# endernewton/tf-faster-rcnn

Hardware: AMD Instinct MI355X
Metric: images/sec (600×1000) ResNet-101 Faster R-CNN at 1/2/4/8 MI355X (higher is better)
Workload: dtype f32 (operands, accumulators, results; GEMMs with Cin, Cout % 128 == 0 form each f32 product from two-piece fp16 operands with an exact power-of-two scale per 128-k block on the fp16 matrix pipe -- 3 MFMAs / product, dropped terms <= 3 * 2^-22, measured error vs float64 below the f32-MFMA kernel's; o

## Files before the change

scratch/wino2_time.py:

```python
import os, sys, statistics
ROOT = os.path.dirname(os.path.dirname(os.path.abspath(__file__)))
sys.path.insert(0, os.path.join(ROOT, "tf-faster-rcnn_amd")); sys.path.insert(0, os.path.join(ROOT, "tf-faster-rcnn_amd", "lib"))
import torch
from frcnn_hip import ops
dev = torch.device("cuda:0")
N, H, W, C = 8, 150, 250, 64
g = torch.Generator(device=dev); g.manual_seed(1)
x = (torch.randn(N, H, W, C, device=dev, generator=g).clamp_(min=0) * torch.exp(torch.rand(N, H, W, 1, device=dev, generator=g) * 4 - 2)).contiguous()
w = (torch.randn(3, 3, C, C, device=dev, generator=g) / 24).cpu().numpy()
u = torch.from_numpy(ops.winograd_filter_transform(w, m=2)).to(dev)
planes = ops.gemm_x3_pack(u)
b = torch.randn(C, device=dev, generator=g)
T = ops.winograd_tiles(N, H, W, 2)
v = torch.empty(16, T, C, device=dev); mm = torch.empty(16, T, C, device=dev)
y0 = torch.empty(N, H, W, C, device=dev); y1 = torch.empty(N, H, W, C, device=dev)
def ev(): return torch.cuda.Event(enable_timing=True)
def timed(fn):
    a, z = ev(), ev(); a.record(); fn(); z.record(); return a, z
R = {"fused": [], "wino_in": [], "gemm_x3": [], "wino_out": []}
for it in range(60):
    e = {}
    e["wino_in"] = timed(lambda: ops.winograd_input_transform(x, v, 2))
    e["gemm_x3"] = timed(lambda: ops.gemm_x3(v, planes, 16, T, C, C, out=mm))
    e["wino_out"] = timed(lambda: ops.winograd_output_transform(mm, b, 1, y0, 2))
    e["fused"] = timed(lambda: ops.winograd2_conv_x3(x, planes, b, 1, y1))
    torch.cuda.synchronize()
    if it >= 10:
        for k, (a, z) in e.items(): R[k].append(a.elapsed_time(z) * 1000.0)
print("bit equal at the bench shape:", torch.equal(y0.view(torch.int32), y1.view(torch.int32)))
for k in ("wino_in", "gemm_x3", "wino_out", "fused"):
    print("%-9s median %7.1f us   min %7.1f us   (n = %d)" % (k, statistics.median(R[k]), min(R[k]), len(R[k])))
print("three launches: median sum %.1f us" % sum(statistics.median(R[k]) for k in ("wino_in", "gemm_x3", "wino_out")))
```

tf-faster-rcnn_amd/csrc/winograd2_fused.hip:

```cpp
#include "common.h"
#include "x3_mma.h"

namespace {

constexpr int W2_RUN = 64, W2_C = 64, W2_NT = 256;
constexpr int W2_V_BYTES = W2_RUN * W2_C * 4;
constexpr int W2_P_BYTES = W2_C * W2_C * 2;
constexpr int W2_U_BYTES = 3 * W2_P_BYTES;
constexpr int W2_LDS = 2 * W2_V_BYTES + 2 * W2_U_BYTES;
constexpr int W2_ITEMS = W2_RUN * (W2_C / 4) / W2_NT;
constexpr unsigned W2_OOB = 0x80000000u;

__device__ __forceinline__ int w2_first(int p) { return p == 0 ? 0 : (p == 2 ? 2 : 1); }
__device__ __forceinline__ int w2_second(int p) { return p == 0 ? 2 : (p == 1 ? 2 : (p == 2 ? 1 : 3)); }

__device__ __forceinline__ float4 w2_pm(const float4 a, const float4 b, bool sub) {
  const float4 c = sub ? make_float4(-b.x, -b.y, -b.z, -b.w) : b;
  return make_float4(a.x + c.x, a.y + c.y, a.z + c.z, a.w + c.w);
}

struct Wino2Params {
  const float* x; const unsigned short* up; const float* bias; float* y;
  int N, H, W, TH, TW, T, act;
};

__global__ __launch_bounds__(W2_NT) void k_wino2_conv_x3(const Wino2Params p) {
  extern __shared__ __attribute__((aligned(16))) char smem[];
  const int tid = threadIdx.x, lane = tid & 63;
  const int wave = __builtin_amdgcn_readfirstlane(tid >> 6);
  const int run0 = blockIdx.x * W2_RUN;
  const int H = p.H, W = p.W;

  const int c4 = tid & 15;
  int off0[W2_ITEMS];
  unsigned ok[W2_ITEMS];
#pragma unroll
  for (int r = 0; r < W2_ITEMS; ++r) {
    const int t = run0 + (tid >> 4) + 16 * r, tc = min(t, p.T - 1);
    const int tx = tc % p.TW, ty = (tc / p.TW) % p.TH, img = tc / (p.TW * p.TH);
    const int ih0 = 2 * ty - 1, iw0 = 2 * tx - 1;
    unsigned m = 0;
#pragma unroll
    for (int i = 0; i < 4; ++i) {
      m |= ((unsigned)(ih0 + i) < (unsigned)H ? 1u : 0u) << i;
      m |= ((unsigned)(iw0 + i) < (unsigned)W ? 1u : 0u) << (4 + i);
    }
    ok[r] = t < p.T ? m : 0u;
    off0[r] = (((img * H + ih0) * W + iw0) * W2_C + c4 * 4) * 4;
  }
  const auto xr = __builtin_amdgcn_make_buffer_rsrc((void*)p.x, 0, p.N * H * W * W2_C * 4, 0x00020000);
  auto tap = [&](int r, int i, int j) {
    const bool in = ((ok[r] >> i) & (ok[r] >> (4 + j)) & 1u) != 0;
    const unsigned o = in ? (unsigned)(off0[r] + (i * W + j) * (W2_C * 4)) : W2_OOB;
    return __builtin_bit_cast(float4, __builtin_amdgcn_raw_buffer_load_b128(xr, (int)o, 0, 0));
  };
  float4 d[W2_ITEMS][4][4];
  auto load_column = [&](int j) {
#pragma unroll
    for (int r = 0; r < W2_ITEMS; ++r)
#pragma unroll
      for (int i = 0; i < 4; ++i) d[r][i][j] = tap(r, i, j);
  };
  load_column(0); load_column(2); load_column(1);
  auto form_v = [&](int xi, int nu, int r, int buf) {
    const int ia = w2_first(xi), ib = w2_second(xi), ja = w2_first(nu), jb = w2_second(nu);
    const bool rsub = xi != 1, csub = nu != 1;
    const float4 ba = w2_pm(d[r][ia][ja], d[r][ib][ja], rsub), bb = w2_pm(d[r][ia][jb], d[r][ib][jb], rsub);
    const int row = (tid >> 4) + 16 * r;
    *(float4*)(smem + buf * W2_V_BYTES + row * (W2_C * 4) + ((c4 ^ (row & 15)) * 16)) = w2_pm(ba, bb, csub);
  };

  const unsigned lds0 = (unsigned)(size_t)(LDS_AS char*)smem;
  int u_lane[2];
#pragma unroll
  for (int t = 0; t < 2; ++t) u_lane[t] = (lane >> 3) * (W2_C * 2) + (((lane & 7) ^ ((4 * t + (lane >> 4)) & 7)) * 16);
  auto load_u = [&](int g, int buf) {
    const char* src = (const char*)p.up + g * W2_U_BYTES + wave * 6 * 1024;
#pragma unroll
    for (int t = 0; t < 6; ++t)
      glds16(src + t * 1024 + u_lane[t & 1], __builtin_amdgcn_readfirstlane(lds0 + 2 * W2_V_BYTES + buf * W2_U_BYTES + (wave * 6 + t) * 1024));
  };

  const int tb = wave >> 1, cb = wave & 1;
  const int frow = lane & 31, khalf = lane >> 5;
  const int a_row = (tb * 32 + frow) * (W2_C * 4), a_sw = frow & 15;
  const int b_row = (cb * 32 + frow) * (W2_C * 2), b_sw = (frow >> 1) & 7;
  f32x16 s0, s1, o[2][2];

  load_u(0, 0);
#pragma unroll
  for (int r = 0; r < W2_ITEMS; ++r) form_v(0, 0, r, 0);
  wait_vmcnt<0>();
  __syncthreads();

#pragma unroll
  for (int nu = 0; nu < 4; ++nu) {
#pragma unroll
    for (int xi = 0; xi < 4; ++xi) {
      const int buf = xi & 1;
      const int nxi = (xi + 1) & 3, nnu = xi == 3 ? nu + 1 : nu;
      const bool more = xi < 3 || nu < 3;
      if (more) load_u(nxi * 4 + nnu, buf ^ 1);
      if (nu == 0 && xi == 3) load_column(3);
      f32x16 acc, acs;
#pragma unroll
      for (int r = 0; r < 16; ++r) { acc[r] = 0.f; acs[r] = 0.f; }
      const char* va = smem + buf * W2_V_BYTES + a_row;
      const char* ub = smem + 2 * W2_V_BYTES + buf * W2_U_BYTES + b_row;
#pragma unroll
      for (int q = 0; q < 4; ++q) {
        bf16x8 ah, am, al;
        const float4 f0 = *(const float4*)(va + (((4 * q + 2 * khalf) ^ a_sw) * 16));
        const float4 f1 = *(const float4*)(va + (((4 * q + 2 * khalf + 1) ^ a_sw) * 16));
        const char* qb = ub + (((2 * q + khalf) ^ b_sw) * 16);
        const bf16x8 bh = __builtin_bit_cast(bf16x8, *(const uint4*)(qb));
        const bf16x8 bm = __builtin_bit_cast(bf16x8, *(const uint4*)(qb + W2_P_BYTES));
        const bf16x8 bl = __builtin_bit_cast(bf16x8, *(const uint4*)(qb + 2 * W2_P_BYTES));
        x3_split8(f0, f1, ah, am, al);
        x3_mma16<6>(ah, am, al, bh, bm, bl, acc, acs);
        if (more) form_v(nxi, nnu, q, buf ^ 1);
      }
      f32x16 m;
#pragma unroll
      for (int r = 0; r < 16; ++r) m[r] = x3_combine_plain(acc[r], acs[r]);
      if (xi == 0) s0 = m;
      if (xi == 1) { s0 = s0 + m; s1 = m; }
      if (xi == 2) { s0 = s0 + m; s1 = s1 - m; }
      if (xi == 3) {
        s1 = s1 - m;
        if (nu == 0) { o[0][0] = s0; o[1][0] = s1; }
        if (nu == 1) { o[0][0] = o[0][0] + s0; o[1][0] = o[1][0] + s1; o[0][1] = s0; o[1][1] = s1; }
        if (nu == 2) { o[0][0] = o[0][0] + s0; o[1][0] = o[1][0] + s1; o[0][1] = o[0][1] - s0; o[1][1] = o[1][1] - s1; }
        if (nu == 3) { o[0][1] = o[0][1] - s0; o[1][1] = o[1][1] - s1; }
      }
      asm volatile("" : "+v"(s0));
      if (xi >= 1) asm volatile("" : "+v"(s1));
      if (xi == 3) {
        if (nu < 3) asm volatile("" : "+v"(o[0][0]), "+v"(o[1][0]));
        if (nu > 0) asm volatile("" : "+v"(o[0][1]), "+v"(o[1][1]));
      }
      wait_vmcnt<0>();
      __syncthreads();
    }
  }

  const int ch = cb * 32 + frow;
  const float bv = p.bias ? p.bias[ch] : 0.f;
  const bool relu = p.act == FRCNN_ACT_RELU;
  int t = run0 + tb * 32 + 4 * khalf;
  int tx = t % p.TW, ty = (t / p.TW) % p.TH, img = t / (p.TW * p.TH);
  auto next_tile = [&]() {
    ++t; ++tx;
    const bool wx = tx == p.TW;
    tx = wx ? 0 : tx; ty += wx ? 1 : 0;
    const bool wy = ty == p.TH;
    ty = wy ? 0 : ty; img += wy ? 1 : 0;
  };
#pragma unroll
  for (int r = 0; r < 16; ++r) {
    if (r) {
#pragma unroll
      for (int k = 0; k < ((r & 3) ? 1 : 5); ++k) next_tile();
    }
    if (t < p.T) {
#pragma unroll
      for (int a = 0; a < 2; ++a)
#pragma unroll
        for (int b = 0; b < 2; ++b) {
          const int oh = 2 * ty + a, ow = 2 * tx + b;
          if (oh >= H || ow >= W) continue;
          float v = o[a][b][r] + bv;
          if (relu) v = act_relu(v);
          p.y[((img * H + oh) * W + ow) * W2_C + ch] = v;
        }
    }
  }
}

}

extern "C" int frcnn_winograd2_conv_x3(const float* x_d, int N, int H, int W, const void* u_planes_d, const float* bias_d, int act,
                                       float* y_d, void* stream) {
  if (!x_d || !u_planes_d || !y_d || N <= 0 || H <= 0 || W <= 0) return FRCNN_E_ARG;
  if (act != FRCNN_ACT_NONE && act != FRCNN_ACT_RELU) return FRCNN_E_UNSUPPORTED;
  if ((long long)N * H * W * W2_C * 4 >= (1ll << 31)) return FRCNN_E_UNSUPPORTED;
  Wino2Params p;
  p.x = x_d; p.up = (const unsigned short*)u_planes_d; p.bias = bias_d; p.y = y_d;
  p.N = N; p.H = H; p.W = W; p.TH = (H + 1) / 2; p.TW = (W + 1) / 2; p.T = N * p.TH * p.TW; p.act = act;
  static KernelOnce once;
  HIP_TRY(kernel_once(once, (const void*)k_wino2_conv_x3, W2_NT, W2_LDS));
  hipLaunchKernelGGL(k_wino2_conv_x3, dim3((unsigned)cdiv(p.T, W2_RUN)), dim3(W2_NT), W2_LDS, (hipStream_t)stream, p);
  LAUNCH_CHECK();
  return FRCNN_OK;
}
```

Before: 563.1.

## Tile fused Winograd F(2,3) conv as 8x8 spatial blocks with LDS halo staging

Each block now owns an 8x8 tile patch of one image rather than a linear run of 64 tiles. It loads the 18x18 input halo once into LDS, split into odd and even column planes, instead of issuing overlapping 4x4 global tap loads per tile. The V operand is split into fp16 hi/mid/lo planes once when written to LDS rather than on every fragment read, and fragments are double-buffered with sched_group_barrier interleaving. Outputs are staged through LDS and written as coalesced float4 rows. This adds LDS pressure and wastes work on edge blocks, and the change also extends the timing script to compare external builds.

```diff
diff --git a/scratch/wino2_time.py b/scratch/wino2_time.py
--- a/scratch/wino2_time.py
+++ b/scratch/wino2_time.py
@@ -1,4 +1,4 @@
-import os, sys, statistics
+import ctypes, os, sys, statistics
 ROOT = os.path.dirname(os.path.dirname(os.path.abspath(__file__)))
 sys.path.insert(0, os.path.join(ROOT, "tf-faster-rcnn_amd")); sys.path.insert(0, os.path.join(ROOT, "tf-faster-rcnn_amd", "lib"))
 import torch
@@ -17,17 +17,29 @@
 def ev(): return torch.cuda.Event(enable_timing=True)
 def timed(fn):
     a, z = ev(), ev(); a.record(); fn(); z.record(); return a, z
-R = {"fused": [], "wino_in": [], "gemm_x3": [], "wino_out": []}
+others = {}
+for path in sys.argv[1:]:
+    L = ctypes.CDLL(os.path.abspath(path)); f = L.frcnn_winograd2_conv_x3; f.restype = ctypes.c_int
+    f.argtypes = [ctypes.c_void_p, ctypes.c_int, ctypes.c_int, ctypes.c_int] + [ctypes.c_void_p] * 2 + [ctypes.c_int] + [ctypes.c_void_p] * 2
+    others["fused@" + os.path.basename(os.path.dirname(os.path.abspath(path)))] = f
+y2 = torch.empty(N, H, W, C, device=dev)
+def other(f):
+    rc = f(x.data_ptr(), N, H, W, planes.data_ptr(), b.data_ptr(), 1, y2.data_ptr(), torch.cuda.current_stream().cuda_stream)
+    assert rc == 0, rc
+R = {k: [] for k in ["fused", "wino_in", "gemm_x3", "wino_out"] + list(others)}
 for it in range(60):
     e = {}
     e["wino_in"] = timed(lambda: ops.winograd_input_transform(x, v, 2))
     e["gemm_x3"] = timed(lambda: ops.gemm_x3(v, planes, 16, T, C, C, out=mm))
     e["wino_out"] = timed(lambda: ops.winograd_output_transform(mm, b, 1, y0, 2))
     e["fused"] = timed(lambda: ops.winograd2_conv_x3(x, planes, b, 1, y1))
+    for k, f in others.items(): e[k] = timed(lambda: other(f))
     torch.cuda.synchronize()
     if it >= 10:
         for k, (a, z) in e.items(): R[k].append(a.elapsed_time(z) * 1000.0)
 print("bit equal at the bench shape:", torch.equal(y0.view(torch.int32), y1.view(torch.int32)))
-for k in ("wino_in", "gemm_x3", "wino_out", "fused"):
+for k, f in others.items():
+    y2.zero_(); other(f); print("%s bit equal to the three launches: %s" % (k, torch.equal(y0.view(torch.int32), y2.view(torch.int32))))
+for k in ["wino_in", "gemm_x3", "wino_out", "fused"] + list(others):
     print("%-9s median %7.1f us   min %7.1f us   (n = %d)" % (k, statistics.median(R[k]), min(R[k]), len(R[k])))
 print("three launches: median sum %.1f us" % sum(statistics.median(R[k]) for k in ("wino_in", "gemm_x3", "wino_out")))
diff --git a/tf-faster-rcnn_amd/csrc/winograd2_fused.hip b/tf-faster-rcnn_amd/csrc/winograd2_fused.hip
--- a/tf-faster-rcnn_amd/csrc/winograd2_fused.hip
+++ b/tf-faster-rcnn_amd/csrc/winograd2_fused.hip
@@ -3,11 +3,17 @@
 
 namespace {
 
-constexpr int W2_RUN = 64, W2_C = 64, W2_NT = 256;
-constexpr int W2_V_BYTES = W2_RUN * W2_C * 4;
+constexpr int W2_BT = 8, W2_RUN = W2_BT * W2_BT, W2_C = 64, W2_NT = 256;
+constexpr int W2_PS = 2 * W2_BT + 2;
 constexpr int W2_P_BYTES = W2_C * W2_C * 2;
-constexpr int W2_U_BYTES = 3 * W2_P_BYTES;
-constexpr int W2_LDS = 2 * W2_V_BYTES + 2 * W2_U_BYTES;
+constexpr int W2_V_BYTES = 3 * W2_P_BYTES, W2_U_BYTES = 3 * W2_P_BYTES;
+constexpr int W2_PLANE = 42 * 1024;
+constexpr int W2_ODD = 0, W2_EVEN = W2_PLANE, W2_V0 = W2_PLANE, W2_U0 = W2_V0 + 2 * W2_V_BYTES;
+constexpr int W2_LDS = W2_PLANE + 2 * W2_V_BYTES + 2 * W2_U_BYTES;
+static_assert(W2_PS * (W2_PS / 2) * W2_C * 4 <= W2_PLANE && W2_PLANE <= 2 * W2_V_BYTES, "the even plane lies inside V[0..1]");
+static_assert(4 * W2_RUN * W2_C * 4 <= W2_LDS, "the block's output pixels fit");
+__device__ __forceinline__ constexpr int w2_v(int buf) { return W2_V0 + buf * W2_V_BYTES; }
+__device__ __forceinline__ constexpr int w2_u(int buf) { return W2_U0 + buf * W2_U_BYTES; }
 constexpr int W2_ITEMS = W2_RUN * (W2_C / 4) / W2_NT;
 constexpr unsigned W2_OOB = 0x80000000u;
 
@@ -21,38 +27,53 @@
 
 struct Wino2Params {
   const float* x; const unsigned short* up; const float* bias; float* y;
-  int N, H, W, TH, TW, T, act;
+  int N, H, W, NBY, NBX, act;
 };
 
 __global__ __launch_bounds__(W2_NT) void k_wino2_conv_x3(const Wino2Params p) {
   extern __shared__ __attribute__((aligned(16))) char smem[];
   const int tid = threadIdx.x, lane = tid & 63;
   const int wave = __builtin_amdgcn_readfirstlane(tid >> 6);
-  const int run0 = blockIdx.x * W2_RUN;
   const int H = p.H, W = p.W;
-
+  const int bx = blockIdx.x % p.NBX, by = (blockIdx.x / p.NBX) % p.NBY, img = blockIdx.x / (p.NBX * p.NBY);
+  const int ih0 = 2 * W2_BT * by - 1, iw0 = 2 * W2_BT * bx - 1;
   const int c4 = tid & 15;
-  int off0[W2_ITEMS];
-  unsigned ok[W2_ITEMS];
-#pragma unroll
-  for (int r = 0; r < W2_ITEMS; ++r) {
-    const int t = run0 + (tid >> 4) + 16 * r, tc = min(t, p.T - 1);
-    const int tx = tc % p.TW, ty = (tc / p.TW) % p.TH, img = tc / (p.TW * p.TH);
-    const int ih0 = 2 * ty - 1, iw0 = 2 * tx - 1;
-    unsigned m = 0;
-#pragma unroll
-    for (int i = 0; i < 4; ++i) {
-      m |= ((unsigned)(ih0 + i) < (unsigned)H ? 1u : 0u) << i;
-      m |= ((unsigned)(iw0 + i) < (unsigned)W ? 1u : 0u) << (4 + i);
+
+  const unsigned lds0 = (unsigned)(size_t)(LDS_AS char*)smem;
+  int u_lane[2];
+#pragma unroll
+  for (int t = 0; t < 2; ++t) u_lane[t] = (lane >> 3) * (W2_C * 2) + (((lane & 7) ^ ((4 * t + (lane >> 4)) & 7)) * 16);
+  auto load_u = [&](int g, int buf) {
+    const char* src = (const char*)p.up + g * W2_U_BYTES + wave * 6 * 1024;
+#pragma unroll
+    for (int t = 0; t < 6; ++t)
+      glds16(src + t * 1024 + u_lane[t & 1], __builtin_amdgcn_readfirstlane(lds0 + w2_u(buf) + (wave * 6 + t) * 1024));
+  };
+  load_u(0, 0);
+
+  {
+    constexpr int CHUNKS = W2_PS * W2_PS * (W2_C / 4), ITS = (CHUNKS + W2_NT - 1) / W2_NT;
+    const auto xr = __builtin_amdgcn_make_buffer_rsrc((void*)p.x, 0, p.N * H * W * W2_C * 4, 0x00020000);
+    float4 px[ITS];
+    int at[ITS];
+#pragma unroll
+    for (int it = 0; it < ITS; ++it) {
+      const int pix = (it * W2_NT + tid) >> 4, pr = pix / W2_PS, pc = pix - pr * W2_PS;
+      const int gh = ih0 + pr, gw = iw0 + pc;
+      const bool in = (unsigned)gh < (unsigned)H && (unsigned)gw < (unsigned)W && pix < W2_PS * W2_PS;
+      const unsigned o = in ? (unsigned)((((img * H + gh) * W + gw) * W2_C + c4 * 4) * 4) : W2_OOB;
+      px[it] = __builtin_bit_cast(float4, __builtin_amdgcn_raw_buffer_load_b128(xr, (int)o, 0, 0));
+      at[it] = ((pc & 1) ? W2_ODD : W2_EVEN) + (pr * (W2_PS / 2) + (pc >> 1)) * (W2_C * 4) + c4 * 16;
     }
-    ok[r] = t < p.T ? m : 0u;
-    off0[r] = (((img * H + ih0) * W + iw0) * W2_C + c4 * 4) * 4;
-  }
-  const auto xr = __builtin_amdgcn_make_buffer_rsrc((void*)p.x, 0, p.N * H * W * W2_C * 4, 0x00020000);
+#pragma unroll
+    for (int it = 0; it < ITS; ++it)
+      if ((it + 1) * W2_NT <= CHUNKS || ((it * W2_NT + tid) >> 4) < W2_PS * W2_PS) *(float4*)(smem + at[it]) = px[it];
+  }
+  __syncthreads();
+
+  const char* taps = smem + (2 * (tid >> 7) * (W2_PS / 2) + ((tid >> 4) & 7)) * (W2_C * 4) + c4 * 16;
   auto tap = [&](int r, int i, int j) {
-    const bool in = ((ok[r] >> i) & (ok[r] >> (4 + j)) & 1u) != 0;
-    const unsigned o = in ? (unsigned)(off0[r] + (i * W + j) * (W2_C * 4)) : W2_OOB;
-    return __builtin_bit_cast(float4, __builtin_amdgcn_raw_buffer_load_b128(xr, (int)o, 0, 0));
+    return *(const float4*)(taps + ((j & 1) ? W2_ODD : W2_EVEN) + ((4 * r + i) * (W2_PS / 2) + (j >> 1)) * (W2_C * 4));
   };
   float4 d[W2_ITEMS][4][4];
   auto load_column = [&](int j) {
@@ -62,34 +83,36 @@
       for (int i = 0; i < 4; ++i) d[r][i][j] = tap(r, i, j);
   };
   load_column(0); load_column(2); load_column(1);
+  __syncthreads();
+  const int v_lane = (tid >> 4) * (W2_C * 2) + (((c4 >> 1) ^ ((tid >> 5) & 7)) * 16) + (c4 & 1) * 8;
   auto form_v = [&](int xi, int nu, int r, int buf) {
     const int ia = w2_first(xi), ib = w2_second(xi), ja = w2_first(nu), jb = w2_second(nu);
     const bool rsub = xi != 1, csub = nu != 1;
-    const float4 ba = w2_pm(d[r][ia][ja], d[r][ib][ja], rsub), bb = w2_pm(d[r][ia][jb], d[r][ib][jb], rsub);
-    const int row = (tid >> 4) + 16 * r;
-    *(float4*)(smem + buf * W2_V_BYTES + row * (W2_C * 4) + ((c4 ^ (row & 15)) * 16)) = w2_pm(ba, bb, csub);
-  };
-
-  const unsigned lds0 = (unsigned)(size_t)(LDS_AS char*)smem;
-  int u_lane[2];
-#pragma unroll
-  for (int t = 0; t < 2; ++t) u_lane[t] = (lane >> 3) * (W2_C * 2) + (((lane & 7) ^ ((4 * t + (lane >> 4)) & 7)) * 16);
-  auto load_u = [&](int g, int buf) {
-    const char* src = (const char*)p.up + g * W2_U_BYTES + wave * 6 * 1024;
-#pragma unroll
-    for (int t = 0; t < 6; ++t)
-      glds16(src + t * 1024 + u_lane[t & 1], __builtin_amdgcn_readfirstlane(lds0 + 2 * W2_V_BYTES + buf * W2_U_BYTES + (wave * 6 + t) * 1024));
+    float4 v[2];
+#pragma unroll
+    for (int e = 0; e < 2; ++e) {
+      const float4 ba = w2_pm(d[r + e][ia][ja], d[r + e][ib][ja], rsub), bb = w2_pm(d[r + e][ia][jb], d[r + e][ib][jb], rsub);
+      v[e] = w2_pm(ba, bb, csub);
+    }
+    bf16x8 h, m, l;
+    x3_split8(v[0], v[1], h, m, l);
+    const uint4 hu = __builtin_bit_cast(uint4, h), mu = __builtin_bit_cast(uint4, m), lu = __builtin_bit_cast(uint4, l);
+    char* at = smem + w2_v(buf) + v_lane + 16 * r * (W2_C * 2);
+    *(uint2*)(at) = make_uint2(hu.x, hu.y);
+    *(uint2*)(at + W2_P_BYTES) = make_uint2(mu.x, mu.y);
+    *(uint2*)(at + 2 * W2_P_BYTES) = make_uint2(lu.x, lu.y);
+    *(uint2*)(at + 16 * (W2_C * 2)) = make_uint2(hu.z, hu.w);
+    *(uint2*)(at + 16 * (W2_C * 2) + W2_P_BYTES) = make_uint2(mu.z, mu.w);
+    *(uint2*)(at + 16 * (W2_C * 2) + 2 * W2_P_BYTES) = make_uint2(lu.z, lu.w);
   };
 
   const int tb = wave >> 1, cb = wave & 1;
   const int frow = lane & 31, khalf = lane >> 5;
-  const int a_row = (tb * 32 + frow) * (W2_C * 4), a_sw = frow & 15;
-  const int b_row = (cb * 32 + frow) * (W2_C * 2), b_sw = (frow >> 1) & 7;
+  const int a_row = (tb * 32 + frow) * (W2_C * 2), b_row = (cb * 32 + frow) * (W2_C * 2), f_sw = (frow >> 1) & 7;
   f32x16 s0, s1, o[2][2];
 
-  load_u(0, 0);
-#pragma unroll
-  for (int r = 0; r < W2_ITEMS; ++r) form_v(0, 0, r, 0);
+#pragma unroll
+  for (int r = 0; r < W2_ITEMS; r += 2) form_v(0, 0, r, 0);
   wait_vmcnt<0>();
   __syncthreads();
 
@@ -105,20 +128,32 @@
       f32x16 acc, acs;
 #pragma unroll
       for (int r = 0; r < 16; ++r) { acc[r] = 0.f; acs[r] = 0.f; }
-      const char* va = smem + buf * W2_V_BYTES + a_row;
-      const char* ub = smem + 2 * W2_V_BYTES + buf * W2_U_BYTES + b_row;
+      const char* va = smem + w2_v(buf) + a_row;
+      const char* ub = smem + w2_u(buf) + b_row;
+      bf16x8 fa[2][3], fb[2][3];
+      auto frags = [&](int q, int s) {
+        const char* qa = va + (((2 * q + khalf) ^ f_sw) * 16), * qb = ub + (((2 * q + khalf) ^ f_sw) * 16);
+#pragma unroll
+        for (int pl = 0; pl < 3; ++pl) {
+          fa[s][pl] = __builtin_bit_cast(bf16x8, *(const uint4*)(qa + pl * W2_P_BYTES));
+          fb[s][pl] = __builtin_bit_cast(bf16x8, *(const uint4*)(qb + pl * W2_P_BYTES));
+        }
+      };
+      frags(0, 0);
 #pragma unroll
       for (int q = 0; q < 4; ++q) {
-        bf16x8 ah, am, al;
-        const float4 f0 = *(const float4*)(va + (((4 * q + 2 * khalf) ^ a_sw) * 16));
-        const float4 f1 = *(const float4*)(va + (((4 * q + 2 * khalf + 1) ^ a_sw) * 16));
-        const char* qb = ub + (((2 * q + khalf) ^ b_sw) * 16);
-        const bf16x8 bh = __builtin_bit_cast(bf16x8, *(const uint4*)(qb));
-        const bf16x8 bm = __builtin_bit_cast(bf16x8, *(const uint4*)(qb + W2_P_BYTES));
-        const bf16x8 bl = __builtin_bit_cast(bf16x8, *(const uint4*)(qb + 2 * W2_P_BYTES));
-        x3_split8(f0, f1, ah, am, al);
-        x3_mma16<6>(ah, am, al, bh, bm, bl, acc, acs);
-        if (more) form_v(nxi, nnu, q, buf ^ 1);
+        if (q < 3) frags(q + 1, (q + 1) & 1);
+        __builtin_amdgcn_sched_barrier(0);
+        x3_mma16<6>(fa[q & 1][0], fa[q & 1][1], fa[q & 1][2], fb[q & 1][0], fb[q & 1][1], fb[q & 1][2], acc, acs);
+        if (more && (q & 1)) form_v(nxi, nnu, q - 1, buf ^ 1);
+        if (more && (q & 1)) {
+#pragma unroll
+          for (int i = 0; i < 6; ++i) {
+            __builtin_amdgcn_sched_group_barrier(0x008, 1, 0);
+            __builtin_amdgcn_sched_group_barrier(0x002, 12, 0);
+          }
+        }
+        __builtin_amdgcn_sched_barrier(0);
       }
       f32x16 m;
 #pragma unroll
@@ -147,33 +182,25 @@
   const int ch = cb * 32 + frow;
   const float bv = p.bias ? p.bias[ch] : 0.f;
   const bool relu = p.act == FRCNN_ACT_RELU;
-  int t = run0 + tb * 32 + 4 * khalf;
-  int tx = t % p.TW, ty = (t / p.TW) % p.TH, img = t / (p.TW * p.TH);
-  auto next_tile = [&]() {
-    ++t; ++tx;
-    const bool wx = tx == p.TW;
-    tx = wx ? 0 : tx; ty += wx ? 1 : 0;
-    const bool wy = ty == p.TH;
-    ty = wy ? 0 : ty; img += wy ? 1 : 0;
-  };
 #pragma unroll
   for (int r = 0; r < 16; ++r) {
-    if (r) {
-#pragma unroll
-      for (int k = 0; k < ((r & 3) ? 1 : 5); ++k) next_tile();
-    }
-    if (t < p.T) {
-#pragma unroll
-      for (int a = 0; a < 2; ++a)
-#pragma unroll
-        for (int b = 0; b < 2; ++b) {
-          const int oh = 2 * ty + a, ow = 2 * tx + b;
-          if (oh >= H || ow >= W) continue;
-          float v = o[a][b][r] + bv;
-          if (relu) v = act_relu(v);
-          p.y[((img * H + oh) * W + ow) * W2_C + ch] = v;
-        }
-    }
+    const int tyl = 4 * tb + (r >> 2), txl = 4 * khalf + (r & 3);
+#pragma unroll
+    for (int a = 0; a < 2; ++a)
+#pragma unroll
+      for (int b = 0; b < 2; ++b) {
+        float v = o[a][b][r] + bv;
+        if (relu) v = act_relu(v);
+        *(float*)(smem + (((2 * tyl + a) * (2 * W2_BT) + 2 * txl + b) * W2_C + ch) * 4) = v;
+      }
+  }
+  __syncthreads();
+  const int ow = 2 * W2_BT * bx + (tid >> 4);
+#pragma unroll
+  for (int k = 0; k < 2 * W2_BT; ++k) {
+    const int oh = 2 * W2_BT * by + k;
+    if (oh < H && ow < W)
+      *(float4*)(p.y + ((img * H + oh) * W + ow) * W2_C + c4 * 4) = *(const float4*)(smem + (k * W2_NT + tid) * 16);
   }
 }
 
@@ -186,10 +213,11 @@
   if ((long long)N * H * W * W2_C * 4 >= (1ll << 31)) return FRCNN_E_UNSUPPORTED;
   Wino2Params p;
   p.x = x_d; p.up = (const unsigned short*)u_planes_d; p.bias = bias_d; p.y = y_d;
-  p.N = N; p.H = H; p.W = W; p.TH = (H + 1) / 2; p.TW = (W + 1) / 2; p.T = N * p.TH * p.TW; p.act = act;
+  p.N = N; p.H = H; p.W = W; p.NBY = cdiv((H + 1) / 2, W2_BT); p.NBX = cdiv((W + 1) / 2, W2_BT); p.act = act;
+  if ((long long)N * p.NBY * p.NBX >= (1ll << 31)) return FRCNN_E_UNSUPPORTED;
   static KernelOnce once;
   HIP_TRY(kernel_once(once, (const void*)k_wino2_conv_x3, W2_NT, W2_LDS));
-  hipLaunchKernelGGL(k_wino2_conv_x3, dim3((unsigned)cdiv(p.T, W2_RUN)), dim3(W2_NT), W2_LDS, (hipStream_t)stream, p);
+  hipLaunchKernelGGL(k_wino2_conv_x3, dim3((unsigned)(N * p.NBY * p.NBX)), dim3(W2_NT), W2_LDS, (hipStream_t)stream, p);
   LAUNCH_CHECK();
   return FRCNN_OK;
 }
```

Result: no change. 566.0, median of 6 (+0.5%).
